# Cappucciyes/ViT-With-OpenCL

Measured on AMD Instinct MI355X. Metric: images/sec ViT-B/16 224x224 bs512, higher is better.
Workload: dtype f32

## Files before the change

### include/kernelHandler.h

```cpp
#ifndef VIT_HIP_KERNELHANDLER_H
#define VIT_HIP_KERNELHANDLER_H

#include <stddef.h>
#include <stdio.h>
#include <stdlib.h>

#ifdef __cplusplus
extern "C" {
#endif

typedef void *vh_stream_t;
typedef void *vh_event_t;

#define VH_CHECK(err)                                                          \
    do {                                                                       \
        int vh_check_err_ = (err);                                             \
        if (vh_check_err_ != 0) {                                              \
            printf("[%s:%d] HIP error %d: %s\n", __FILE__, __LINE__,           \
                   vh_check_err_, vh_last_error());                            \
            exit(EXIT_FAILURE);                                                \
        }                                                                      \
    } while (0)

int vh_device_count(void);
// ... 89 lines not shown
int vh_launch_attention_planes_f16(vh_stream_t s, const void *qkv_planes_f16, void *output, int output_planes,
                                   int n_images, int tokens, int embed_dim, int num_heads);
int vh_launch_attention_planes_f16_hd80(vh_stream_t s, const void *qkv_planes_f16, float *output, int n_images,
                                        int tokens, int embed_dim, int num_heads);
int vh_launch_attention_planes_f16_hd80_operand(vh_stream_t s, const void *qkv_planes_f16, void *output, void *out_scales,
                                                int output_kind, int n_images, int tokens, int embed_dim, int num_heads);
int vh_launch_attention_long(vh_stream_t s, const void *qkv_planes, int parts, float *output, int n_images, int tokens,
                             int embed_dim, int num_heads);
int vh_launch_linear_p3(vh_stream_t s, void *output, int output_planes, const void *weight_planes,
                        const void *input_planes, const float *bias, int rowA, int colA, int colB,
                        int doGelu, const float *residual);
int vh_launch_linear_p3_cols(vh_stream_t s, void *output, int output_planes, const void *weight_planes, int w_features,
                             const void *input_planes, const float *bias, int rowA, int colA, int colB);
int vh_launch_attention_planes_cls(vh_stream_t s, const void *qkv_planes, const void *q_cls_planes, void *out_cls_planes,
                                   int n_images, int tokens, int embed_dim, int num_heads);

int vh_launch_split2h_planes(vh_stream_t s, const float *weight, void *planes, int rows, int cols, float scale);
int vh_launch_linear_h2(vh_stream_t s, float *output, const void *weight_planes, float weight_scale,
                        const float *input, const float *bias, int rowA, int colA, int colB,
                        int doGelu, const float *residual);
int vh_launch_attention_h2(vh_stream_t s, const float *qkv, float *output, int n_images, int tokens,
                           int embed_dim, int num_heads);

int vh_launch_attention(vh_stream_t s, const float *qkv, float *output, int n_images,
                        int tokens, int embed_dim, int num_heads);
enum { VH_ATTN_NATIVE = 0, VH_ATTN_FP16 = 1, VH_ATTN_FP16X2 = 2, VH_ATTN_SPLIT3 = 3 };
enum { VH_ATTN_AUTO = 0, VH_ATTN_STREAMING = 1 };
int vh_launch_attention_rows(vh_stream_t s, const float *qkv, void *output, int out_kind, int arith, int kernel, int n_images,
                             int tokens, int embed_dim, int num_heads);

// ... 168 lines not shown
```

### vit-with-opencl_amd/csrc/ViT_hip.c

```c
#include "ViT_opencl.h"
#include "kernel_limits.h"
#include "vit_ingest.h"
#include "vit_multi.h"
#include "vit_pipeline.h"
#include "vit_plan.h"
#include "vit_planes_file.h"
#include "vit_requests.h"

#include <math.h>
#include <stdint.h>
#include <stdio.h>
#include <stdlib.h>
#include <string.h>
#include <time.h>

#define TRY(expr)                 \
    do {                          \
        int try_rc_ = (expr);     \
        if (try_rc_ != 0) {       \
            rc = try_rc_;         \
            goto fail;            \
        }                         \
    } while (0)

// ... 558 lines not shown
    return rc;
}

static int layer_f32_planes_attention(vit_hip_ctx *ctx, vh_stream_t s, int n, int l, int timed)
{
    int rc = 0;
    const vit_config *c = &ctx->cfg;
    const int E = c->embed_dim, T = ctx->plan.tokens, rows = n * T, fold = ctx->plan.ln_fold;
    float **lw = layer_tensors(ctx, l);
    const struct operand *op = ctx->op + 4 * l;
    const int planes_attn = ctx->plan.qkv_form == VH_QKV_PLANES3;
    OP_T(timed, VIT_OP_QKV, fold ? vh_launch_linear_p3_norm(s, ctx->qkv, planes_attn, op[0].w, ctx->y, ctx->stats, op[0].colsum, op[0].bias_folded, c->eps, rows, E, 3 * E, 0)
                                 : vh_launch_linear_p3(s, ctx->qkv, planes_attn, op[0].w, ctx->y, lw[3], rows, E, 3 * E, 0, NULL));
    if (timed)
        TRY(attention_tap(ctx, s, n, l));
    OP_T(timed, VIT_OP_ATTENTION, ctx->plan.attn_form == ATTN_HD64 ? vh_launch_attention_planes(s, ctx->qkv, ctx->attn, n, T, E, c->num_heads)
                                  : (rc = ctx->plan.attn_form == ATTN_LONG ? vh_launch_attention_long(s, ctx->qkv, 3, ctx->hid, n, T, E, c->num_heads)
                                                                      : attention_rows(ctx, s, ctx->hid, VH_ATTN_SPLIT3, n)) != 0 ? rc
                                  : vh_launch_split3_rows(s, ctx->hid, ctx->attn, rows, E));
    return 0;
fail:
    return rc;
}

static int layer_f32_planes_tail(vit_hip_ctx *ctx, vh_stream_t s, int n, int l, int timed)
{
    int rc = 0;
    const vit_config *c = &ctx->cfg;
    const int E = c->embed_dim, F = c->mlp_hidden, rows = n * ctx->plan.tokens, fold = ctx->plan.ln_fold, last = l == c->depth - 1;
    float **lw = layer_tensors(ctx, l);
    const struct operand *op = ctx->op + 4 * l;
// ... 44 lines not shown
    if (!fold)
        OP(VIT_OP_LAYER_NORM, vh_launch_layer_norm_p3(s, ctx->x, lw[0], lw[1], ctx->y, rows, E, E, c->eps));
    if (last && cls_only) {
        size_t off[3], q_off;
        plan_cls_only_scratch(c, n, off);
        plan_cls_query_scratch(c, n, &q_off);
        char *scratch = (char *)ctx->qkv;
        float *x_cls = (float *)scratch;
        char *attn_cls = scratch + off[0], *y_cls = scratch + off[1], *hid_cls = scratch + off[2], *q_cls = scratch + q_off;
        const int cls_query = ctx->plan.cls_query && !attention_tap_reads(ctx, l);
        if (cls_query) {
            char *kv = scratch + (size_t)rows * E * 6;
            OP(VIT_OP_QKV, (rc = vh_launch_linear_p3_cols(s, kv, 1, (const char *)op[0].w + (size_t)E * 64, 3 * E, ctx->y, lw[3] + E, rows, E, 2 * E)) != 0 ? rc :
                           (rc = vh_launch_gather_rows(s, ctx->y, y_cls, 3 * (E / 32), rows, n, 64, T)) != 0 ? rc :
                           vh_launch_linear_p3_cols(s, q_cls, 1, op[0].w, 3 * E, y_cls, lw[3], n, E, E));
            OP(VIT_OP_ATTENTION, vh_launch_attention_planes_cls(s, ctx->qkv, q_cls, attn_cls, n, T, E, c->num_heads));
        } else {
            TRY(layer_f32_planes_attention(ctx, s, n, l, 1));
        }
        OP(VIT_OP_OUT_PROJ_CLS, (rc = cls_query ? 0 : vh_launch_gather_rows(s, ctx->attn, attn_cls, 3 * (E / 32), rows, n, 64, T)) != 0 ? rc :
                                (rc = vh_launch_gather_rows(s, ctx->x, x_cls, 1, rows, n, 4 * E, T)) != 0 ? rc :
                                vh_launch_linear_p3(s, x_cls, 0, op[1].w, attn_cls, lw[5], n, E, E, 0, x_cls));
        OP(VIT_OP_LAYER_NORM, vh_launch_layer_norm_p3(s, x_cls, lw[6], lw[7], y_cls, n, E, E, c->eps));
        OP(VIT_OP_FC1_CLS, vh_launch_linear_p3(s, hid_cls, 1, op[2].w, y_cls, lw[9], n, E, F, 1, NULL));
        OP(VIT_OP_FC2_CLS, vh_launch_linear_p3(s, x_cls, 0, op[3].w, hid_cls, lw[11], n, F, E, 0, x_cls));
        *cls_rows = cls_query ? 2 : 1;
        return 0;
    }
    TRY(layer_f32_planes_attention(ctx, s, n, l, 1));
    return layer_f32_planes_tail(ctx, s, n, l, 1);
fail:
// ... 771 lines not shown
```

### vit-with-opencl_amd/csrc/attention_p3.hip

```cpp
#include "kernelHandler.h"
#include "kernel_limits.h"
#include "vit_kernels.h"
#include "fp32_split.h"
#include "gemm_common.h"

namespace {

constexpr int HD = 64;
constexpr int MAX_LDS = KL_LDS_BYTES;
constexpr int MAX_ROWS = KL_ATTN_HD64_MAX_TOKENS;
static_assert(2 * 2 * 3 * MAX_ROWS * 64 <= MAX_LDS && MAX_ROWS % 16 == 0 && MAX_ROWS <= 32 * 7, "the rows of launch_k and launch_t");

typedef const __attribute__((address_space(1))) void *gptr_t;
typedef __attribute__((address_space(3))) void *lptr_t;
typedef short s16x4 __attribute__((ext_vector_type(4)));

template <int NKT, int NPL, int OUTK, bool CLSQ = false>
__global__ __launch_bounds__(64 * NKT) void attention_p3_kernel(const char *__restrict__ qkv3, char *__restrict__ out3,
                                                               unsigned char *__restrict__ aux,
                                                               int T, int E, int H, int n_items, int RB)
{
    static_assert((NPL == 3 && OUTK == 3) || (NPL == 1 && (OUTK == 4 || OUTK == 0 || OUTK == 8)), "parts / output kind");
    static_assert(!CLSQ || OUTK == 3, "the class-query variant runs on the exact planes");
    unsigned char *const out_scales = aux;
    typedef typename PartT<NPL>::type part_t;
    constexpr int NT = NPL == 3 ? 6 : 1;
    extern __shared__ __attribute__((aligned(16))) char smem[];
    const int slot = 2 * NPL * RB * 64;
    char *Kb = smem, *Vb = smem + slot;

    const int tid = threadIdx.x, lane = tid & 63;
    const int wave = __builtin_amdgcn_readfirstlane(tid >> 6);
    const int lr = lane & 31, lh = lane >> 5;
    const int E32 = E >> 5, rb16 = RB >> 4, pieces = 2 * NPL * rb16;
    const size_t prow = (size_t)(n_items / H) * T;
// ... 99 lines not shown
                        __builtin_amdgcn_sched_group_barrier(0x008, 2, 0);
                    }
                    __builtin_amdgcn_sched_barrier(0);
                }
            }
        }

        __syncthreads();
        if (next < n_items) {
            dma(next, 1, Kb);
            if (computes)
                load_q(next);
        }

        if (computes) {
#pragma unroll
            for (int r = 0; r < 16; ++r) {
                const int key = 32 * (NKT - 1) + (r & 3) + 8 * (r >> 2) + 4 * lh;
                s[NKT - 1][r] = key < T ? s[NKT - 1][r] : -INFINITY;
            }
            float mx = -INFINITY;
#pragma unroll
            for (int j = 0; j < NKT; ++j)
#pragma unroll
                for (int r = 0; r < 16; ++r)
                    mx = fmaxf(mx, s[j][r]);
            mx = fmaxf(mx, __shfl_xor(mx, 32));
            const float c1 = 1.44269504088896340736f / sqrtf((float)HD);
            const float c2 = -mx * c1;
            float sum = 0.0f;
#pragma unroll
            for (int j = 0; j < NKT; ++j)
#pragma unroll
                for (int r = 0; r < 16; ++r) {
                    const float e = __builtin_amdgcn_exp2f(__builtin_fmaf(s[j][r], c1, c2));
                    s[j][r] = e;
                    sum += e;
                }
            sum += __shfl_xor(sum, 32);
            const float inv_sum = 1.0f / sum;
#pragma unroll
            for (int j = 0; j < NKT; ++j)
#pragma unroll
                for (int r = 0; r < 16; ++r)
                    s[j][r] = s[j][r] * inv_sum;

            f32x16 o[2];
#pragma unroll
            for (int r = 0; r < 16; ++r) {
                o[0][r] = 0.0f;
                o[1][r] = 0.0f;
            }
            part_t vq[2][NPL], pp[NPL];
            auto read_v = [&](part_t (&v3)[NPL], int f) {
                const int j = f >> 2, t = (f >> 1) & 1, dt = f & 1;
                const int r0 = (j == NKT - 1) ? min(32 * j + 16 * t, RB - 16) : 32 * j + 16 * t;
#pragma unroll
                for (int o3 = 0; o3 < NPL; ++o3) {
                    const int pl = (NPL - o3) % NPL;
                    const char *vp = Vb + (dt * NPL + pl) * RB * 64 + r0 * 64 + vofs;
                    const s16x4 lo = __builtin_amdgcn_ds_read_tr16_b64_v4i16((__attribute__((address_space(3))) s16x4 *)(vp));
                    const s16x4 hi = __builtin_amdgcn_ds_read_tr16_b64_v4i16((__attribute__((address_space(3))) s16x4 *)(vp + 8 * 64));
                    typedef short s16x8 __attribute__((ext_vector_type(8)));
                    v3[pl] = __builtin_bit_cast(part_t, s16x8{lo[0], lo[1], lo[2], lo[3], hi[0], hi[1], hi[2], hi[3]});
                }
            };
            read_v(vq[0], 0);
#pragma unroll
            for (int f = 0; f < 4 * NKT; ++f) {
                const int j = f >> 2, t = (f >> 1) & 1, dt = f & 1;
                if (f + 1 < 4 * NKT)
                    read_v(vq[(f + 1) & 1], f + 1);
                if (dt == 0)
                    split_parts(f32x4{s[j][8 * t], s[j][8 * t + 1], s[j][8 * t + 2], s[j][8 * t + 3]},
                                f32x4{s[j][8 * t + 4], s[j][8 * t + 5], s[j][8 * t + 6], s[j][8 * t + 7]}, pp);
                if (!(j == NKT - 1 && 32 * j + 16 * t >= T)) {
#pragma unroll
                    for (int tt = 0; tt < NT; ++tt)
                        o[dt] = mfma_part(vq[f & 1][term_w<NPL>(tt)], pp[term_a<NPL>(tt)], o[dt]);
                }
            }

            if (CLSQ ? lr == 0 : q < T) {
                typedef unsigned u32x2 __attribute__((ext_vector_type(2)));
                typedef unsigned u32x4 __attribute__((ext_vector_type(4)));
                constexpr int OPL = OUTK == 3 ? 3 : 1;
#pragma unroll
                for (int dt = 0; dt < 2; ++dt) {
                    if (OUTK == 0) {
                        float *row = reinterpret_cast<float *>(out3) + ((size_t)b * T + q) * E + h * HD + 32 * dt + 4 * lh;
// ... 46 lines not shown
                    for (int pl = 0; pl < OPL; ++pl)
#pragma unroll
                        for (int g = 0; g < 4; g += 2) {
                            const auto r0 = __builtin_amdgcn_permlane32_swap(pg[g][pl][0], pg[g + 1][pl][0], false, false);
                            const auto r1 = __builtin_amdgcn_permlane32_swap(pg[g][pl][1], pg[g + 1][pl][1], false, false);
                            *reinterpret_cast<u32x4 *>(d3 + (size_t)pl * orows * 64 + 16 * g) = u32x4{r0[0], r1[0], r0[1], r1[1]};
                        }
                }
            }
        }

        __syncthreads();
    }
}

template <int NKT, int NPL, int OUTK, bool CLSQ>
int launch_k(hipStream_t st, const char *qkv3, char *out3, unsigned char *aux, int n_images, int T, int E, int H)
{
    const int RB = (T + 15) / 16 * 16;
    const size_t lds = (size_t)2 * 2 * NPL * RB * 64;
    VH_SET_LDS_ONCE((attention_p3_kernel<NKT, NPL, OUTK, CLSQ>), MAX_LDS);
    const int num_cus = vh_device_cus(vh_current_device());
    const int n_items = n_images * H;
    const int grid = n_items < num_cus ? n_items : num_cus;
    hipLaunchKernelGGL((attention_p3_kernel<NKT, NPL, OUTK, CLSQ>), dim3(grid), dim3(64 * NKT), lds, st, qkv3, out3, aux, T, E, H, n_items, RB);
    VH_LAUNCH_CHECK("attention_p3_kernel");
    return 0;
}


template <int NPL, int OUTK, bool CLSQ = false>
int launch_t(hipStream_t st, const char *in, char *out, unsigned char *out_scales, int n_images, int tokens, int embed_dim, int num_heads)
{
    switch ((tokens + 31) / 32) {
    case 1: return launch_k<1, NPL, OUTK, CLSQ>(st, in, out, out_scales, n_images, tokens, embed_dim, num_heads);
    case 2: return launch_k<2, NPL, OUTK, CLSQ>(st, in, out, out_scales, n_images, tokens, embed_dim, num_heads);
    case 3: return launch_k<3, NPL, OUTK, CLSQ>(st, in, out, out_scales, n_images, tokens, embed_dim, num_heads);
    case 4: return launch_k<4, NPL, OUTK, CLSQ>(st, in, out, out_scales, n_images, tokens, embed_dim, num_heads);
    case 5: return launch_k<5, NPL, OUTK, CLSQ>(st, in, out, out_scales, n_images, tokens, embed_dim, num_heads);
    case 6: return launch_k<6, NPL, OUTK, CLSQ>(st, in, out, out_scales, n_images, tokens, embed_dim, num_heads);
    default: return launch_k<7, NPL, OUTK, CLSQ>(st, in, out, out_scales, n_images, tokens, embed_dim, num_heads);
    }
}

int check_args(const char *who, const void *in, const void *out, int n_images, int tokens, int embed_dim, int num_heads)
{
    if (!in || !out)
        return vh_fail(1, "%s: null pointer argument", who);
    if (n_images <= 0 || tokens <= 0 || num_heads <= 0 || embed_dim != num_heads * HD || tokens > MAX_ROWS)
        return vh_fail(1, "%s: needs head_dim 64 and 1 <= tokens <= %d (n=%d tokens=%d embed=%d heads=%d)", who,
                       MAX_ROWS, n_images, tokens, embed_dim, num_heads);
    if ((((uintptr_t)in | (uintptr_t)out) & 15) != 0)
        return vh_fail(1, "%s: pointers must be 16-byte aligned", who);
    return 0;
}

// ... 7 lines not shown
    return launch_t<3, 3>((hipStream_t)s, static_cast<const char *>(qkv_planes), static_cast<char *>(out_planes), nullptr,
                          n_images, tokens, embed_dim, num_heads);
}

extern "C" int vh_launch_attention_planes_cls(vh_stream_t s, const void *qkv_planes, const void *q_cls_planes, void *out_cls_planes,
                                              int n_images, int tokens, int embed_dim, int num_heads)
{
    if (int rc = check_args("vh_launch_attention_planes_cls", qkv_planes, out_cls_planes, n_images, tokens, embed_dim, num_heads))
        return rc;
    if (!q_cls_planes || ((uintptr_t)q_cls_planes & 15) != 0)
        return vh_fail(1, "vh_launch_attention_planes_cls: q_cls_planes must be a 16-byte aligned pointer");
    return launch_t<3, 3, true>((hipStream_t)s, static_cast<const char *>(qkv_planes), static_cast<char *>(out_cls_planes),
                                static_cast<unsigned char *>(const_cast<void *>(q_cls_planes)), n_images, tokens, embed_dim, num_heads);
}

extern "C" int vh_launch_attention_planes_f16(vh_stream_t s, const void *qkv_planes_f16, void *output, int output_planes,
                                              int n_images, int tokens, int embed_dim, int num_heads)
{
    if (int rc = check_args("vh_launch_attention_planes_f16", qkv_planes_f16, output, n_images, tokens, embed_dim, num_heads))
        return rc;
    const char *in = static_cast<const char *>(qkv_planes_f16);
    char *out = static_cast<char *>(output);
    return output_planes ? launch_t<1, 4>((hipStream_t)s, in, out, nullptr, n_images, tokens, embed_dim, num_heads)
                         : launch_t<1, 0>((hipStream_t)s, in, out, nullptr, n_images, tokens, embed_dim, num_heads);
}

extern "C" int vh_launch_attention_planes_f16_mx(vh_stream_t s, const void *qkv_planes_f16, void *out_values, void *out_scales,
                                                 int n_images, int tokens, int embed_dim, int num_heads)
{
    if (int rc = check_args("vh_launch_attention_planes_f16_mx", qkv_planes_f16, out_values, n_images, tokens, embed_dim, num_heads))
// ... 7 lines not shown
```

### vit-with-opencl_amd/csrc/kernel_limits.h

```cpp
#ifndef VIT_KERNEL_LIMITS_H
#define VIT_KERNEL_LIMITS_H

#include "kernelHandler.h"

#include <stddef.h>

#ifdef __cplusplus
#define KL_FN static constexpr
#else
#define KL_FN static inline
#endif

enum { KL_LDS_BYTES = 160 * 1024 };

enum {
    KL_ATTN_HD64_MAX_TOKENS = 208,
    KL_ATTN_HD80_MAX_TOKENS = 272,
    KL_ATTN_STREAMING_MAX_TOKENS = 512
};
KL_FN int kl_attn_long_head_dim_ok(int head_dim) { return head_dim == 64 || head_dim == 80; }

enum { KL_LN_PLANES_ROWS = 16, KL_LN_PLANES_MAX_EMBED = 2048 };
KL_FN int kl_layer_norm_planes_max_embed(int parts)
{
    if (parts != 1 && parts != 3)
        return 0;
    const int by_lds = KL_LDS_BYTES / (parts * KL_LN_PLANES_ROWS * 64) * 32;
    return by_lds < KL_LN_PLANES_MAX_EMBED ? by_lds : KL_LN_PLANES_MAX_EMBED;
}

enum { KL_FOLD_GROUP = 128, KL_FOLD_MAX_GROUPS = 16 };

enum {
// ... 89 lines not shown
```

### vit-with-opencl_amd/csrc/vit_plan.c

```c
#include "vit_plan.h"
#include "vit_ingest.h"
#include "kernel_limits.h"

#include <stdio.h>
#include <stdlib.h>
#include <string.h>

void plan_env_parse(struct plan_env *env, const char *const v[PLAN_ENV_COUNT])
{
    const char *const p = v[PLAN_ENV_PRECISION], *const fold = v[PLAN_ENV_LN_FOLD], *const attn = v[PLAN_ENV_ATTN];
    env->precision = (p && p[0] == 'b') ? VIT_PRECISION_BF16_GEMM
                   : (p && strncmp(p, "fp16x2", 6) == 0) ? VIT_PRECISION_F32_FP16X2
                   : (p && strncmp(p, "fp8", 3) == 0) ? VIT_PRECISION_FP8_GEMM : VIT_PRECISION_F32;
    env->p3_off = v[PLAN_ENV_P3] && v[PLAN_ENV_P3][0] == '0';
    env->fp32_native = v[PLAN_ENV_GEMM_FP32] && v[PLAN_ENV_GEMM_FP32][0] == 'n';
    env->ln_fold = (fold && fold[0] == '0') ? 0 : (fold && fold[0] == '1') ? 1 : -1;
    env->last_layer_cls = v[PLAN_ENV_LAST_LAYER] && strcmp(v[PLAN_ENV_LAST_LAYER], "cls") == 0;
    env->last_layer_full = v[PLAN_ENV_LAST_LAYER] && strcmp(v[PLAN_ENV_LAST_LAYER], "full") == 0;
    env->last_layer_all_queries = v[PLAN_ENV_LAST_LAYER] && strcmp(v[PLAN_ENV_LAST_LAYER], "all_queries") == 0;
    env->attn_long = attn && strcmp(attn, "long") == 0;
    env->attn_tiled = attn && attn[0] == 't';
}

void plan_env_read(struct plan_env *env)
{
    const char *const values[PLAN_ENV_COUNT] = {getenv("VIT_HIP_PRECISION"), getenv("VIT_HIP_P3"), getenv("VIT_HIP_GEMM_FP32"),
                                                getenv("VIT_HIP_LN_FOLD"), getenv("VIT_HIP_LAST_LAYER"), getenv("VIT_HIP_ATTN")};
    plan_env_parse(env, values);
}

static size_t max_of(size_t a, size_t b) { return a > b ? a : b; }

size_t plan_cls_only_scratch(const vit_config *cfg, int n, size_t off[3])
{
    const size_t rows = (size_t)n, E = (size_t)cfg->embed_dim, F = (size_t)cfg->mlp_hidden;
    size_t o[3];
    o[0] = align_up(rows * E * 4, 256);
    o[1] = o[0] + align_up(rows * E * 6, 256);
    o[2] = o[1] + align_up(rows * E * 6, 256);
    if (off)
        memcpy(off, o, sizeof o);
    return o[2] + rows * F * 6;
}
// ... 158 lines not shown
    plan->qkv_form = plan->attn_form == ATTN_STREAMING ? VH_QKV_ROWS_F32 : reduced ? VH_QKV_PLANES_F16 : VH_QKV_PLANES3;
    plan->weight_planes = weight_planes;
    plan->operand_bytes = precision == VIT_PRECISION_BF16_GEMM ? 2 : precision == VIT_PRECISION_FP8_GEMM ? 1
                        : precision == VIT_PRECISION_F32_FP16X2 ? 4 : weight_planes ? 6 : 0;
    plan->operand_scales = precision == VIT_PRECISION_FP8_GEMM;
    plan->conv_parts = reduced ? 1 : weight_planes ? 3 : 0;
    plan->planes_patch_embed = plan->ln_fold || use_p3 || reduced;
    plan->act_bytes = use_p3 ? 6 : (int)sizeof(float);
    plan_layout(plan, cfg, NULL, NULL, NULL, plan->slab_bytes);
    plan_arena(plan, cfg, max_batch);
    plan->cls_only_ok = use_p3 && !ln_fold && T >= 4 && plan_cls_only_scratch(cfg, max_batch, NULL) <= plan->qkv_bytes;
    plan->last_layer_lazy = plan->cls_only_ok && !env->last_layer_full;
    plan->cls_query = plan->last_layer_lazy && !env->last_layer_all_queries && plan->attn_form == ATTN_HD64 &&
                      plan->qkv_form == VH_QKV_PLANES3 &&
                      22 * (size_t)E + 6 * (size_t)F + 5 * 256 <= (size_t)T * (size_t)E * 6;
    return 0;
}
```

### vit-with-opencl_amd/csrc/vit_plan.h

```cpp
#ifndef VIT_PLAN_H
#define VIT_PLAN_H

#include "ViT_opencl.h"

#include <stddef.h>

struct operand
{
    void *w;
    void *scales;
    float pair_scale;
    float *colsum, *bias_folded;
};

enum { SLAB_F32, SLAB_OPERAND, SLAB_CONV, SLAB_FOLD, N_SLABS };

enum { ATTN_STREAMING, ATTN_HD64, ATTN_HD80, ATTN_LONG };

enum { MAX_DEPTH = 256, MAX_TENSORS = 4 + 12 * MAX_DEPTH + 4 };

static inline int plan_operand_tensor(int m)
{
    static const int big[4] = {2, 4, 8, 10};
    return 4 + 12 * (m / 4) + big[m % 4];
}

struct plan_env
{
    int precision;
    int p3_off;
    int fp32_native;
    int ln_fold;
    int last_layer_cls;
    int last_layer_full;
    int last_layer_all_queries;
    int attn_long;
    int attn_tiled;
};
enum { PLAN_ENV_PRECISION, PLAN_ENV_P3, PLAN_ENV_GEMM_FP32, PLAN_ENV_LN_FOLD, PLAN_ENV_LAST_LAYER, PLAN_ENV_ATTN, PLAN_ENV_COUNT };
void plan_env_parse(struct plan_env *env, const char *const values[PLAN_ENV_COUNT]);
void plan_env_read(struct plan_env *env);

struct vit_plan
{
    int precision;
    int ln_fold;
    int use_p3;
    int cls_only_last;
    int attn_form;
    int fp32_native;
    int attn_rows_streaming;
    int tokens;
    int qkv_form;
    int weight_planes;
    int operand_bytes;
    int operand_scales;
    int conv_parts;
    int planes_patch_embed;
    int act_bytes;
    int cls_only_ok;
    int last_layer_lazy;
    int cls_query;
    size_t slab_bytes[N_SLABS];
    size_t x_bytes, y_bytes, attn_bytes, qkv_bytes, ws_bytes, stats_bytes;
    size_t crop_off;
    size_t e_scales_off, hid_scales_off;
};

int plan_make(struct vit_plan *plan, const vit_config *cfg, int n_tensors, int max_batch, int precision, int ln_fold,
              const struct plan_env *env);

void plan_layout(const struct vit_plan *plan, const vit_config *cfg, void *const slabs[N_SLABS], float **w, struct operand *op,
                 size_t bytes[N_SLABS]);

size_t plan_cls_only_scratch(const vit_config *cfg, int n, size_t off[3]);
size_t plan_cls_query_scratch(const vit_config *cfg, int n, size_t *q_off);

// ... 2 lines not shown
```

### vit-with-opencl_amd/host/abi.py

```python
from __future__ import annotations

import ctypes as C

P = C.POINTER
i, u, l, sz, ull, f, d = C.c_int, C.c_uint, C.c_long, C.c_size_t, C.c_ulonglong, C.c_float, C.c_double
p, s = C.c_void_p, C.c_char_p
voidp = p
f32p = fp = P(f)
pp, fpp, ip, lp, dp, szp, u8p = P(p), P(fp), P(i), P(l), P(d), P(sz), P(C.c_ubyte)

STRUCTS = {}
ENUMS = []


def mirrors(ctype: str):
    def register(cls):
        STRUCTS[ctype] = cls
        return cls
    return register


def enum(prefix: str, mapping: dict, names: dict | None = None) -> dict:
    ENUMS.append((prefix, mapping, names))
    return mapping


FP32_MATH = enum("VH_FP32_", {"split3": 0, "native": 1})
ATTN_ARITH = enum("VH_ATTN_", {"native": 0, "fp16": 1, "fp16x2": 2, "split3": 3})
ATTN_KERNEL = enum("VH_ATTN_", {"auto": 0, "streaming": 1})
QKV_FORMS = enum("VH_QKV_", {"rows_f32": 0, "planes3": 1, "planes_f16": 2})
TOPK_SCORES = enum("VIT_TOPK_", {"probs": 0, "logits": 1})
GALLERY_DTYPES = enum("VH_GALLERY_", {"f32": 0, "bf16": 1})
GALLERY_MAX_SPLITS, GALLERY_ROW_TILE = 1024, 128
enum("VH_GALLERY_", {"max_splits": GALLERY_MAX_SPLITS, "row_tile": GALLERY_ROW_TILE})
DENSE_MAX_LABELS, DENSE_MAX_GRID, DENSE_TOKEN_TILE = 256, 64, 128
enum("VH_DENSE_", {"max_labels": DENSE_MAX_LABELS, "max_grid": DENSE_MAX_GRID, "token_tile": DENSE_TOKEN_TILE})
STITCH_BLOCK, STITCH_MAX_SIDE = 16, 16384
enum("VH_STITCH_", {"block": STITCH_BLOCK, "max_side": STITCH_MAX_SIDE})
POS_MODES = enum("VH_POS_", {"bicubic": 0, "bilinear": 1})
enum("VIT_POS_", POS_MODES)

PRECISIONS = enum("VIT_PRECISION_", {"f32": 0, "bf16": 1, "fp8": 2, "f32_fp16x2": 3},
                  names={"bf16": "VIT_PRECISION_BF16_GEMM", "fp8": "VIT_PRECISION_FP8_GEMM"})
PIXEL_LAYOUTS = enum("VIT_PIXELS_", {"hwc": 0, "chw": 1})
# ... 197 lines not shown
        _fn("vh_launch_merge_rows", p, p, p, i, i, i),
        _fn("vh_layer_norm_planes_max_embed", i),
        _fn("vh_launch_layer_norm_planes", p, p, p, p, p, i, i, i, l, d),
        _fn("vh_launch_attention_planes_bf16", p, p, p, i, i, i, i),
        _fn("vh_launch_linear_planes", p, p, i, p, p, i, p, i, i, i, i, p),
        _fn("vh_launch_layer_norm_p3", p, p, p, p, p, i, i, l, d),
        _fn("vh_launch_attention_p3", p, p, p, i, i, i, i),
        _fn("vh_launch_attention_planes", p, p, p, i, i, i, i),
        _fn("vh_launch_attention_planes_f16", p, p, p, i, i, i, i, i),
        _fn("vh_launch_attention_planes_f16_hd80", p, p, p, i, i, i, i),
        _fn("vh_launch_attention_planes_f16_hd80_operand", p, p, p, p, i, i, i, i, i),
        _fn("vh_launch_attention_long", p, p, i, p, i, i, i, i),
        _fn("vh_launch_linear_p3", p, p, i, p, p, p, i, i, i, i, p),
        _fn("vh_launch_linear_p3_cols", p, p, i, p, i, p, p, i, i, i),
        _fn("vh_launch_attention_planes_cls", p, p, p, p, i, i, i, i),
        _fn("vh_launch_split2h_planes", p, p, p, i, i, f),
        _fn("vh_launch_linear_h2", p, p, p, f, p, p, i, i, i, i, p),
        _fn("vh_launch_attention_h2", p, p, p, i, i, i, i),
        _fn("vh_launch_attention", p, p, p, i, i, i, i),
        _fn("vh_launch_attention_rows", p, p, p, i, i, i, i, i, i, i),
        _fn("vh_launch_gather_rows", p, p, p, i, i, i, i, i),
        _fn("vh_launch_softmax", p, p, p, i, i),
        _fn("vh_launch_topk", p, p, i, i, i, i, p, p),
        _fn("vh_cls_attention_head_dim_ok", i),
        _fn("vh_launch_cls_attention", p, p, i, i, i, i, i, i, i, p, p),
        _fn("vh_rollout_workspace", i, i, ret=sz),
        _fn("vh_rollout_max_tokens", i),
        _fn("vh_launch_rollout_step", p, p, i, i, i, i, i, p, p, p),
        _fn("vh_launch_rollout_read", p, p, i, i, p),
        _fn("vh_launch_attention_f16", p, p, p, i, i, i, i),
# ... 149 lines not shown
```

Before: 6529.

## Skip masked key groups in attention softmax and add one-wave CLS attention kernel

Attention softmax now checks the count of live keys in the last 32-key tile and skips max, exp, scale and split work for groups that are fully past the token count. This is the default path unless VIT_HIP_ATTN_MASKED=all is set. A new single-wave persistent kernel handles the last layer's class-token query. It stages V through LDS with transposed reads and prefetches the next head, and it becomes the default unless VIT_HIP_CLS_ATTN=workgroup is set. The change cuts wasted ALU work on padded keys and over-provisioned workgroups for the CLS-only layer, at the cost of more code paths and branches.

```diff
diff --git a/include/kernelHandler.h b/include/kernelHandler.h
--- a/include/kernelHandler.h
+++ b/include/kernelHandler.h
@@ -127,6 +127,12 @@
                              const void *input_planes, const float *bias, int rowA, int colA, int colB);
 int vh_launch_attention_planes_cls(vh_stream_t s, const void *qkv_planes, const void *q_cls_planes, void *out_cls_planes,
                                    int n_images, int tokens, int embed_dim, int num_heads);
+enum {
+    VH_ATTN_CLS_WORKGROUP = 1,
+    VH_ATTN_EVERY_GROUP = 2
+};
+int vh_launch_attention_planes_forms(vh_stream_t s, const void *qkv_planes, const void *q_cls_planes, void *out_planes,
+                                     int n_images, int tokens, int embed_dim, int num_heads, unsigned forms);
 
 int vh_launch_split2h_planes(vh_stream_t s, const float *weight, void *planes, int rows, int cols, float scale);
 int vh_launch_linear_h2(vh_stream_t s, float *output, const void *weight_planes, float weight_scale,
diff --git a/vit-with-opencl_amd/csrc/ViT_hip.c b/vit-with-opencl_amd/csrc/ViT_hip.c
--- a/vit-with-opencl_amd/csrc/ViT_hip.c
+++ b/vit-with-opencl_amd/csrc/ViT_hip.c
@@ -596,7 +596,7 @@
                                  : vh_launch_linear_p3(s, ctx->qkv, planes_attn, op[0].w, ctx->y, lw[3], rows, E, 3 * E, 0, NULL));
     if (timed)
         TRY(attention_tap(ctx, s, n, l));
-    OP_T(timed, VIT_OP_ATTENTION, ctx->plan.attn_form == ATTN_HD64 ? vh_launch_attention_planes(s, ctx->qkv, ctx->attn, n, T, E, c->num_heads)
+    OP_T(timed, VIT_OP_ATTENTION, ctx->plan.attn_form == ATTN_HD64 ? vh_launch_attention_planes_forms(s, ctx->qkv, NULL, ctx->attn, n, T, E, c->num_heads, ctx->plan.attn_forms)
                                   : (rc = ctx->plan.attn_form == ATTN_LONG ? vh_launch_attention_long(s, ctx->qkv, 3, ctx->hid, n, T, E, c->num_heads)
                                                                       : attention_rows(ctx, s, ctx->hid, VH_ATTN_SPLIT3, n)) != 0 ? rc
                                   : vh_launch_split3_rows(s, ctx->hid, ctx->attn, rows, E));
@@ -671,7 +671,7 @@
             OP(VIT_OP_QKV, (rc = vh_launch_linear_p3_cols(s, kv, 1, (const char *)op[0].w + (size_t)E * 64, 3 * E, ctx->y, lw[3] + E, rows, E, 2 * E)) != 0 ? rc :
                            (rc = vh_launch_gather_rows(s, ctx->y, y_cls, 3 * (E / 32), rows, n, 64, T)) != 0 ? rc :
                            vh_launch_linear_p3_cols(s, q_cls, 1, op[0].w, 3 * E, y_cls, lw[3], n, E, E));
-            OP(VIT_OP_ATTENTION, vh_launch_attention_planes_cls(s, ctx->qkv, q_cls, attn_cls, n, T, E, c->num_heads));
+            OP(VIT_OP_ATTENTION, vh_launch_attention_planes_forms(s, ctx->qkv, q_cls, attn_cls, n, T, E, c->num_heads, ctx->plan.attn_forms));
         } else {
             TRY(layer_f32_planes_attention(ctx, s, n, l, 1));
         }
diff --git a/vit-with-opencl_amd/csrc/attention_p3.hip b/vit-with-opencl_amd/csrc/attention_p3.hip
--- a/vit-with-opencl_amd/csrc/attention_p3.hip
+++ b/vit-with-opencl_amd/csrc/attention_p3.hip
@@ -4,6 +4,8 @@
 #include "fp32_split.h"
 #include "gemm_common.h"
 
+#include <utility>
+
 namespace {
 
 constexpr int HD = 64;
@@ -15,10 +17,96 @@
 typedef __attribute__((address_space(3))) void *lptr_t;
 typedef short s16x4 __attribute__((ext_vector_type(4)));
 
+template <int NKT>
+__device__ __forceinline__ void softmax_columns(f32x16 (&s)[NKT], int T, int lh, int live)
+{
+    constexpr int L = NKT - 1;
+    const float c1 = 1.44269504088896340736f / sqrtf((float)HD);
+    float mx = -INFINITY;
+    auto mask_max = [&](int g) {
+#pragma unroll
+        for (int r = 4 * g; r < 4 * g + 4; ++r) {
+            const int key = 32 * L + (r & 3) + 8 * (r >> 2) + 4 * lh;
+            s[L][r] = key < T ? s[L][r] : -INFINITY;
+            mx = fmaxf(mx, s[L][r]);
+        }
+    };
+#pragma unroll
+    for (int j = 0; j < L; ++j)
+#pragma unroll
+        for (int r = 0; r < 16; ++r)
+            mx = fmaxf(mx, s[j][r]);
+    mask_max(0);
+    if (8 < live) {
+        mask_max(1);
+        if (16 < live) {
+            mask_max(2);
+            if (24 < live)
+                mask_max(3);
+        }
+    }
+    mx = fmaxf(mx, __shfl_xor(mx, 32));
+    const float c2 = -mx * c1;
+    float sum = 0.0f;
+    auto exp_sum = [&](int j, int g) {
+#pragma unroll
+        for (int r = 4 * g; r < 4 * g + 4; ++r) {
+            const float e = __builtin_amdgcn_exp2f(__builtin_fmaf(s[j][r], c1, c2));
+            s[j][r] = e;
+            sum += e;
+        }
+    };
+#pragma unroll
+    for (int j = 0; j < L; ++j)
+#pragma unroll
+        for (int g = 0; g < 4; ++g)
+            exp_sum(j, g);
+    exp_sum(L, 0);
+    if (8 < live) {
+        exp_sum(L, 1);
+        if (16 < live) {
+            exp_sum(L, 2);
+            if (24 < live)
+                exp_sum(L, 3);
+        }
+    }
+    sum += __shfl_xor(sum, 32);
+    const float inv_sum = 1.0f / sum;
+    auto scale = [&](int j, int g) {
+#pragma unroll
+        for (int r = 4 * g; r < 4 * g + 4; ++r)
+            s[j][r] = s[j][r] * inv_sum;
+    };
+#pragma unroll
+    for (int j = 0; j < L; ++j)
+#pragma unroll
+        for (int g = 0; g < 4; ++g)
+            scale(j, g);
+    scale(L, 0);
+    if (8 < live) {
+        scale(L, 1);
+        if (16 < live) {
+            scale(L, 2);
+            if (24 < live)
+                scale(L, 3);
+        }
+    }
+}
+
+template <int NKT, int NPL>
+__device__ __forceinline__ void split_p(const f32x16 (&s)[NKT], int j, int t, int live, typename PartT<NPL>::type (&pp)[NPL])
+{
+    const f32x4 lo = f32x4{s[j][8 * t], s[j][8 * t + 1], s[j][8 * t + 2], s[j][8 * t + 3]};
+    if (j == NKT - 1 && 8 * (2 * t + 1) >= live)
+        split_parts(lo, f32x4{0.0f, 0.0f, 0.0f, 0.0f}, pp);
+    else
+        split_parts(lo, f32x4{s[j][8 * t + 4], s[j][8 * t + 5], s[j][8 * t + 6], s[j][8 * t + 7]}, pp);
+}
+
 template <int NKT, int NPL, int OUTK, bool CLSQ = false>
 __global__ __launch_bounds__(64 * NKT) void attention_p3_kernel(const char *__restrict__ qkv3, char *__restrict__ out3,
                                                                unsigned char *__restrict__ aux,
-                                                               int T, int E, int H, int n_items, int RB)
+                                                               int T, int E, int H, int n_items, int RB, int live)
 {
     static_assert((NPL == 3 && OUTK == 3) || (NPL == 1 && (OUTK == 4 || OUTK == 0 || OUTK == 8)), "parts / output kind");
     static_assert(!CLSQ || OUTK == 3, "the class-query variant runs on the exact planes");
@@ -148,36 +236,7 @@
         }
 
         if (computes) {
-#pragma unroll
-            for (int r = 0; r < 16; ++r) {
-                const int key = 32 * (NKT - 1) + (r & 3) + 8 * (r >> 2) + 4 * lh;
-                s[NKT - 1][r] = key < T ? s[NKT - 1][r] : -INFINITY;
-            }
-            float mx = -INFINITY;
-#pragma unroll
-            for (int j = 0; j < NKT; ++j)
-#pragma unroll
-                for (int r = 0; r < 16; ++r)
-                    mx = fmaxf(mx, s[j][r]);
-            mx = fmaxf(mx, __shfl_xor(mx, 32));
-            const float c1 = 1.44269504088896340736f / sqrtf((float)HD);
-            const float c2 = -mx * c1;
-            float sum = 0.0f;
-#pragma unroll
-            for (int j = 0; j < NKT; ++j)
-#pragma unroll
-                for (int r = 0; r < 16; ++r) {
-                    const float e = __builtin_amdgcn_exp2f(__builtin_fmaf(s[j][r], c1, c2));
-                    s[j][r] = e;
-                    sum += e;
-                }
-            sum += __shfl_xor(sum, 32);
-            const float inv_sum = 1.0f / sum;
-#pragma unroll
-            for (int j = 0; j < NKT; ++j)
-#pragma unroll
-                for (int r = 0; r < 16; ++r)
-                    s[j][r] = s[j][r] * inv_sum;
+            softmax_columns<NKT>(s, T, lh, live);
 
             f32x16 o[2];
 #pragma unroll
@@ -205,9 +264,8 @@
                 const int j = f >> 2, t = (f >> 1) & 1, dt = f & 1;
                 if (f + 1 < 4 * NKT)
                     read_v(vq[(f + 1) & 1], f + 1);
-                if (dt == 0)
-                    split_parts(f32x4{s[j][8 * t], s[j][8 * t + 1], s[j][8 * t + 2], s[j][8 * t + 3]},
-                                f32x4{s[j][8 * t + 4], s[j][8 * t + 5], s[j][8 * t + 6], s[j][8 * t + 7]}, pp);
+                if (dt == 0 && !(j == NKT - 1 && 16 * t >= live))
+                    split_p<NKT, NPL>(s, j, t, live, pp);
                 if (!(j == NKT - 1 && 32 * j + 16 * t >= T)) {
 #pragma unroll
                     for (int tt = 0; tt < NT; ++tt)
@@ -284,32 +342,232 @@
     }
 }
 
+template <class F, int... I>
+__device__ __forceinline__ void static_for_each(F &&f, std::integer_sequence<int, I...>)
+{
+    (f(std::integral_constant<int, I>{}), ...);
+}
+template <int N, class F>
+__device__ __forceinline__ void static_for(F &&f)
+{
+    static_for_each(f, std::make_integer_sequence<int, N>{});
+}
+
+constexpr int CW_LDS = KL_ATTN_CLS_WAVE_LDS_BYTES;
+static_assert(CW_LDS == 2 * 3 * 32 * 64, "one 32-key tile of V: [d tile][part][32 rows][64 B]");
+
+template <int NKT>
+__global__ __launch_bounds__(64) void attention_p3_cls_wave_kernel(const char *__restrict__ qkv3, char *__restrict__ out3,
+                                                                   const char *__restrict__ qcls, int T, int E, int H,
+                                                                   int n_items, int live)
+{
+    constexpr int NPL = 3, NT = 6, NF = NKT * (HD / 16);
+    constexpr int KR = NF < 7 ? NF + 1 : 7;
+    constexpr int VR = NKT < 2 ? NKT : 2;
+    typedef bf16x8 part_t;
+    __shared__ __attribute__((aligned(16))) char vtile[CW_LDS];
+
+    const int lane = threadIdx.x, lr = lane & 31, lh = lane >> 5;
+    const int E32 = E >> 5;
+    const size_t orows = (size_t)(n_items / H), prow = orows * T;
+    const int vofs = (4 * lh + ((lane & 15) >> 2)) * 64 + ((lane & 16) + 4 * (lane & 3)) * 2;
+
+    f32x4 qraw[HD / 16][NPL];
+    auto load_q = [&](int it) {
+        const int b = it / H, h = it - b * H;
+#pragma unroll
+        for (int g = 0; g < HD / 16; ++g)
+#pragma unroll
+            for (int pl = 0; pl < NPL; ++pl)
+                qraw[g][pl] = *reinterpret_cast<const f32x4 *>(
+                    qcls + ((size_t)((2 * h + (g >> 1)) * NPL + pl) * orows + b) * 64 + 16 * (2 * (g & 1) + lh));
+    };
+    part_t kp[KR][NPL];
+    auto load_k = [&](part_t (&k3)[NPL], int it, int f) {
+        const int b = it / H, h = it - b * H;
+        const int j = f / (HD / 16), g = f % (HD / 16);
+        const size_t row = (size_t)b * T + min(32 * j + lr, T - 1);
+#pragma unroll
+        for (int o = 0; o < NPL; ++o) {
+            const int pl = (NPL - o) % NPL;
+            k3[pl] = __builtin_bit_cast(part_t, *reinterpret_cast<const f32x4 *>(
+                         qkv3 + ((size_t)((E32 + 2 * h + (g >> 1)) * NPL + pl) * prow + row) * 64 + 16 * (2 * (g & 1) + lh)));
+        }
+    };
+    auto load_head = [&](int it) {
+        load_q(it);
+#pragma unroll
+        for (int f = 0; f < KR - 1; ++f)
+            load_k(kp[f], it, f);
+    };
+
+    int item = blockIdx.x;
+    load_head(item);
+    for (;;) {
+        const int b = item / H, h = item - b * H;
+        const int next = item + (int)gridDim.x;
+
+        part_t qp[HD / 16][NPL];
+#pragma unroll
+        for (int g = 0; g < HD / 16; ++g)
+#pragma unroll
+            for (int pl = 0; pl < NPL; ++pl)
+                qp[g][pl] = __builtin_bit_cast(part_t, lr == 0 ? qraw[g][pl] : f32x4{0.0f, 0.0f, 0.0f, 0.0f});
+
+        f32x16 s[NKT];
+#pragma unroll
+        for (int f = 0; f < NF; ++f) {
+            const int j = f / (HD / 16), g = f % (HD / 16);
+            if (g == 0) {
+#pragma unroll
+                for (int r = 0; r < 16; ++r)
+                    s[j][r] = 0.0f;
+            }
+            if (f + KR - 1 < NF)
+                load_k(kp[(f + KR - 1) % KR], item, f + KR - 1);
+            __builtin_amdgcn_sched_barrier(0);
+#pragma unroll
+            for (int t = 0; t < NT; ++t)
+                s[j] = mfma_part(kp[f % KR][term_w<NPL>(t)], qp[g][term_a<NPL>(t)], s[j]);
+            __builtin_amdgcn_sched_barrier(0);
+        }
+
+        f32x4 vst[VR][12];
+        auto load_v = [&](int j) {
+#pragma unroll
+            for (int p = 0; p < 12; ++p) {
+                const int r = 32 * j + 16 * (p & 1) + (lane >> 2);
+                vst[j % VR][p] = *reinterpret_cast<const f32x4 *>(
+                    qkv3 + ((size_t)((2 * E32 + 2 * h) * NPL + (p >> 1)) * prow + (size_t)b * T + min(r, T - 1)) * 64 + 16 * (lane & 3));
+            }
+        };
+        auto store_v = [&](int j) {
+#pragma unroll
+            for (int p = 0; p < 12; ++p)
+                *reinterpret_cast<f32x4 *>(vtile + p * 1024 + lane * 16) = vst[j % VR][p];
+        };
+#pragma unroll
+        for (int j = 0; j < VR; ++j)
+            load_v(j);
+        load_head(next < n_items ? next : item);
+        __builtin_amdgcn_sched_barrier(0);
+
+        softmax_columns<NKT>(s, T, lh, live);
+
+        f32x16 o[2];
+#pragma unroll
+        for (int r = 0; r < 16; ++r) {
+            o[0][r] = 0.0f;
+            o[1][r] = 0.0f;
+        }
+        part_t vq[2][NPL], pp[NPL];
+        auto read_v = [&](part_t (&v3)[NPL], int f) {
+            const int t = (f >> 1) & 1, dt = f & 1;
+#pragma unroll
+            for (int o3 = 0; o3 < NPL; ++o3) {
+                const int pl = (NPL - o3) % NPL;
+                const char *vp = vtile + (dt * NPL + pl) * 2048 + 16 * t * 64 + vofs;
+                const s16x4 lo = __builtin_amdgcn_ds_read_tr16_b64_v4i16((__attribute__((address_space(3))) s16x4 *)(vp));
+                const s16x4 hi = __builtin_amdgcn_ds_read_tr16_b64_v4i16((__attribute__((address_space(3))) s16x4 *)(vp + 8 * 64));
+                typedef short s16x8 __attribute__((ext_vector_type(8)));
+                v3[pl] = __builtin_bit_cast(part_t, s16x8{lo[0], lo[1], lo[2], lo[3], hi[0], hi[1], hi[2], hi[3]});
+            }
+        };
+        store_v(0);
+        if (VR < NKT)
+            load_v(VR);
+        read_v(vq[0], 0);
+        static_for<4 * NKT>([&](auto step) __attribute__((always_inline)) {
+            constexpr int f = decltype(step)::value, j = f >> 2, t = (f >> 1) & 1, dt = f & 1;
+            if (f + 1 < 4 * NKT) {
+                if ((f & 3) == 3) {
+                    store_v(j + 1);
+                    if (j + 1 + VR < NKT)
+                        load_v(j + 1 + VR);
+                }
+                read_v(vq[(f + 1) & 1], f + 1);
+            }
+            if (dt == 0 && !(j == NKT - 1 && 16 * t >= live))
+                split_p<NKT, NPL>(s, j, t, live, pp);
+            if (!(j == NKT - 1 && 32 * j + 16 * t >= T)) {
+#pragma unroll
+                for (int tt = 0; tt < NT; ++tt)
+                    o[dt] = mfma_part(vq[f & 1][term_w<NPL>(tt)], pp[term_a<NPL>(tt)], o[dt]);
+            }
+        });
+
+        if (lr == 0) {
+            typedef unsigned u32x2 __attribute__((ext_vector_type(2)));
+            typedef unsigned u32x4 __attribute__((ext_vector_type(4)));
+#pragma unroll
+            for (int dt = 0; dt < 2; ++dt) {
+                u32x2 pg[4][NPL];
+#pragma unroll
+                for (int g = 0; g < 4; ++g) {
+                    bf16x4 part[3];
+                    split4(f32x4{o[dt][4 * g], o[dt][4 * g + 1], o[dt][4 * g + 2], o[dt][4 * g + 3]}, part[0], part[1], part[2]);
+#pragma unroll
+                    for (int pl = 0; pl < NPL; ++pl)
+                        pg[g][pl] = __builtin_bit_cast(u32x2, part[pl]);
+                }
+                char *d3 = out3 + ((size_t)(2 * h + dt) * NPL * orows + (size_t)b) * 64 + 16 * lh;
+#pragma unroll
+                for (int pl = 0; pl < NPL; ++pl)
+#pragma unroll
+                    for (int g = 0; g < 4; g += 2) {
+                        const auto r0 = __builtin_amdgcn_permlane32_swap(pg[g][pl][0], pg[g + 1][pl][0], false, false);
+                        const auto r1 = __builtin_amdgcn_permlane32_swap(pg[g][pl][1], pg[g + 1][pl][1], false, false);
+                        *reinterpret_cast<u32x4 *>(d3 + (size_t)pl * orows * 64 + 16 * g) = u32x4{r0[0], r1[0], r0[1], r1[1]};
+                    }
+            }
+        }
+        if (next >= n_items)
+            break;
+        item = next;
+    }
+}
+
+template <int NKT>
+int launch_cls_wave(hipStream_t st, const char *qkv3, char *out3, const char *qcls, int n_images, int T, int E, int H, int live)
+{
+    const int n_items = n_images * H, waves = vh_device_cus(vh_current_device()) * KL_ATTN_CLS_WAVES_PER_CU;
+    hipLaunchKernelGGL((attention_p3_cls_wave_kernel<NKT>), dim3(n_items < waves ? n_items : waves), dim3(64), 0, st, qkv3, out3, qcls,
+                       T, E, H, n_items, live);
+    VH_LAUNCH_CHECK("attention_p3_cls_wave_kernel");
+    return 0;
+}
+
 template <int NKT, int NPL, int OUTK, bool CLSQ>
-int launch_k(hipStream_t st, const char *qkv3, char *out3, unsigned char *aux, int n_images, int T, int E, int H)
-{
+int launch_k(hipStream_t st, const char *qkv3, char *out3, unsigned char *aux, int n_images, int T, int E, int H, unsigned forms)
+{
+    const int live = (forms & VH_ATTN_EVERY_GROUP) ? 32 : T - 32 * (NKT - 1);
+    if constexpr (CLSQ)
+        if (!(forms & VH_ATTN_CLS_WORKGROUP))
+            return launch_cls_wave<NKT>(st, qkv3, out3, reinterpret_cast<const char *>(aux), n_images, T, E, H, live);
     const int RB = (T + 15) / 16 * 16;
     const size_t lds = (size_t)2 * 2 * NPL * RB * 64;
     VH_SET_LDS_ONCE((attention_p3_kernel<NKT, NPL, OUTK, CLSQ>), MAX_LDS);
     const int num_cus = vh_device_cus(vh_current_device());
     const int n_items = n_images * H;
     const int grid = n_items < num_cus ? n_items : num_cus;
-    hipLaunchKernelGGL((attention_p3_kernel<NKT, NPL, OUTK, CLSQ>), dim3(grid), dim3(64 * NKT), lds, st, qkv3, out3, aux, T, E, H, n_items, RB);
+    hipLaunchKernelGGL((attention_p3_kernel<NKT, NPL, OUTK, CLSQ>), dim3(grid), dim3(64 * NKT), lds, st, qkv3, out3, aux, T, E, H, n_items, RB, live);
     VH_LAUNCH_CHECK("attention_p3_kernel");
     return 0;
 }
 
 
 template <int NPL, int OUTK, bool CLSQ = false>
-int launch_t(hipStream_t st, const char *in, char *out, unsigned char *out_scales, int n_images, int tokens, int embed_dim, int num_heads)
+int launch_t(hipStream_t st, const char *in, char *out, unsigned char *out_scales, int n_images, int tokens, int embed_dim, int num_heads,
+             unsigned forms = 0)
 {
     switch ((tokens + 31) / 32) {
-    case 1: return launch_k<1, NPL, OUTK, CLSQ>(st, in, out, out_scales, n_images, tokens, embed_dim, num_heads);
-    case 2: return launch_k<2, NPL, OUTK, CLSQ>(st, in, out, out_scales, n_images, tokens, embed_dim, num_heads);
-    case 3: return launch_k<3, NPL, OUTK, CLSQ>(st, in, out, out_scales, n_images, tokens, embed_dim, num_heads);
-    case 4: return launch_k<4, NPL, OUTK, CLSQ>(st, in, out, out_scales, n_images, tokens, embed_dim, num_heads);
-    case 5: return launch_k<5, NPL, OUTK, CLSQ>(st, in, out, out_scales, n_images, tokens, embed_dim, num_heads);
-    case 6: return launch_k<6, NPL, OUTK, CLSQ>(st, in, out, out_scales, n_images, tokens, embed_dim, num_heads);
-    default: return launch_k<7, NPL, OUTK, CLSQ>(st, in, out, out_scales, n_images, tokens, embed_dim, num_heads);
+    case 1: return launch_k<1, NPL, OUTK, CLSQ>(st, in, out, out_scales, n_images, tokens, embed_dim, num_heads, forms);
+    case 2: return launch_k<2, NPL, OUTK, CLSQ>(st, in, out, out_scales, n_images, tokens, embed_dim, num_heads, forms);
+    case 3: return launch_k<3, NPL, OUTK, CLSQ>(st, in, out, out_scales, n_images, tokens, embed_dim, num_heads, forms);
+    case 4: return launch_k<4, NPL, OUTK, CLSQ>(st, in, out, out_scales, n_images, tokens, embed_dim, num_heads, forms);
+    case 5: return launch_k<5, NPL, OUTK, CLSQ>(st, in, out, out_scales, n_images, tokens, embed_dim, num_heads, forms);
+    case 6: return launch_k<6, NPL, OUTK, CLSQ>(st, in, out, out_scales, n_images, tokens, embed_dim, num_heads, forms);
+    default: return launch_k<7, NPL, OUTK, CLSQ>(st, in, out, out_scales, n_images, tokens, embed_dim, num_heads, forms);
     }
 }
 
@@ -347,6 +605,21 @@
                                 static_cast<unsigned char *>(const_cast<void *>(q_cls_planes)), n_images, tokens, embed_dim, num_heads);
 }
 
+extern "C" int vh_launch_attention_planes_forms(vh_stream_t s, const void *qkv_planes, const void *q_cls_planes, void *out_planes,
+                                                int n_images, int tokens, int embed_dim, int num_heads, unsigned forms)
+{
+    if (int rc = check_args("vh_launch_attention_planes_forms", qkv_planes, out_planes, n_images, tokens, embed_dim, num_heads))
+        return rc;
+    if (((uintptr_t)q_cls_planes & 15) != 0 || (forms & ~(unsigned)(VH_ATTN_CLS_WORKGROUP | VH_ATTN_EVERY_GROUP)) != 0)
+        return vh_fail(1, "vh_launch_attention_planes_forms: q_cls_planes must be 16-byte aligned and forms a set of VH_ATTN_* (%u)", forms);
+    const char *in = static_cast<const char *>(qkv_planes);
+    char *out = static_cast<char *>(out_planes);
+    if (!q_cls_planes)
+        return launch_t<3, 3>((hipStream_t)s, in, out, nullptr, n_images, tokens, embed_dim, num_heads, forms);
+    return launch_t<3, 3, true>((hipStream_t)s, in, out, static_cast<unsigned char *>(const_cast<void *>(q_cls_planes)), n_images, tokens,
+                                embed_dim, num_heads, forms);
+}
+
 extern "C" int vh_launch_attention_planes_f16(vh_stream_t s, const void *qkv_planes_f16, void *output, int output_planes,
                                               int n_images, int tokens, int embed_dim, int num_heads)
 {
diff --git a/vit-with-opencl_amd/csrc/kernel_limits.h b/vit-with-opencl_amd/csrc/kernel_limits.h
--- a/vit-with-opencl_amd/csrc/kernel_limits.h
+++ b/vit-with-opencl_amd/csrc/kernel_limits.h
@@ -17,6 +17,12 @@
     KL_ATTN_HD64_MAX_TOKENS = 208,
     KL_ATTN_HD80_MAX_TOKENS = 272,
     KL_ATTN_STREAMING_MAX_TOKENS = 512
+};
+enum {
+    KL_ATTN_CLS_WAVE_LDS_BYTES = 2 * 3 * 32 * 64,
+    KL_SIMDS_PER_CU = 4,
+    KL_ATTN_CLS_WAVES_PER_CU = KL_LDS_BYTES / KL_ATTN_CLS_WAVE_LDS_BYTES < KL_SIMDS_PER_CU ? KL_LDS_BYTES / KL_ATTN_CLS_WAVE_LDS_BYTES
+                                                                                           : KL_SIMDS_PER_CU
 };
 KL_FN int kl_attn_long_head_dim_ok(int head_dim) { return head_dim == 64 || head_dim == 80; }
 
diff --git a/vit-with-opencl_amd/csrc/vit_plan.c b/vit-with-opencl_amd/csrc/vit_plan.c
--- a/vit-with-opencl_amd/csrc/vit_plan.c
+++ b/vit-with-opencl_amd/csrc/vit_plan.c
@@ -20,13 +20,22 @@
     env->last_layer_all_queries = v[PLAN_ENV_LAST_LAYER] && strcmp(v[PLAN_ENV_LAST_LAYER], "all_queries") == 0;
     env->attn_long = attn && strcmp(attn, "long") == 0;
     env->attn_tiled = attn && attn[0] == 't';
+    env->cls_attn_workgroup = env->attn_masked_all = 0;
+}
+
+void plan_env_parse_forms(struct plan_env *env, const char *const v[PLAN_FORM_COUNT])
+{
+    env->cls_attn_workgroup = v[PLAN_FORM_CLS_ATTN] && strcmp(v[PLAN_FORM_CLS_ATTN], "workgroup") == 0;
+    env->attn_masked_all = v[PLAN_FORM_ATTN_MASKED] && strcmp(v[PLAN_FORM_ATTN_MASKED], "all") == 0;
 }
 
 void plan_env_read(struct plan_env *env)
 {
     const char *const values[PLAN_ENV_COUNT] = {getenv("VIT_HIP_PRECISION"), getenv("VIT_HIP_P3"), getenv("VIT_HIP_GEMM_FP32"),
                                                 getenv("VIT_HIP_LN_FOLD"), getenv("VIT_HIP_LAST_LAYER"), getenv("VIT_HIP_ATTN")};
+    const char *const forms[PLAN_FORM_COUNT] = {getenv("VIT_HIP_CLS_ATTN"), getenv("VIT_HIP_ATTN_MASKED")};
     plan_env_parse(env, values);
+    plan_env_parse_forms(env, forms);
 }
 
 static size_t max_of(size_t a, size_t b) { return a > b ? a : b; }
@@ -215,5 +224,8 @@
     plan->cls_query = plan->last_layer_lazy && !env->last_layer_all_queries && plan->attn_form == ATTN_HD64 &&
                       plan->qkv_form == VH_QKV_PLANES3 &&
                       22 * (size_t)E + 6 * (size_t)F + 5 * 256 <= (size_t)T * (size_t)E * 6;
+    if (plan->attn_form == ATTN_HD64 && plan->qkv_form == VH_QKV_PLANES3)
+        plan->attn_forms = (plan->cls_query && env->cls_attn_workgroup ? VH_ATTN_CLS_WORKGROUP : 0u) |
+                           (env->attn_masked_all ? VH_ATTN_EVERY_GROUP : 0u);
     return 0;
 }
diff --git a/vit-with-opencl_amd/csrc/vit_plan.h b/vit-with-opencl_amd/csrc/vit_plan.h
--- a/vit-with-opencl_amd/csrc/vit_plan.h
+++ b/vit-with-opencl_amd/csrc/vit_plan.h
@@ -36,9 +36,13 @@
     int last_layer_all_queries;
     int attn_long;
     int attn_tiled;
+    int cls_attn_workgroup;
+    int attn_masked_all;
 };
 enum { PLAN_ENV_PRECISION, PLAN_ENV_P3, PLAN_ENV_GEMM_FP32, PLAN_ENV_LN_FOLD, PLAN_ENV_LAST_LAYER, PLAN_ENV_ATTN, PLAN_ENV_COUNT };
 void plan_env_parse(struct plan_env *env, const char *const values[PLAN_ENV_COUNT]);
+enum { PLAN_FORM_CLS_ATTN, PLAN_FORM_ATTN_MASKED, PLAN_FORM_COUNT };
+void plan_env_parse_forms(struct plan_env *env, const char *const values[PLAN_FORM_COUNT]);
 void plan_env_read(struct plan_env *env);
 
 struct vit_plan
@@ -61,6 +65,7 @@
     int cls_only_ok;
     int last_layer_lazy;
     int cls_query;
+    unsigned attn_forms;
     size_t slab_bytes[N_SLABS];
     size_t x_bytes, y_bytes, attn_bytes, qkv_bytes, ws_bytes, stats_bytes;
     size_t crop_off;
diff --git a/vit-with-opencl_amd/host/abi.py b/vit-with-opencl_amd/host/abi.py
--- a/vit-with-opencl_amd/host/abi.py
+++ b/vit-with-opencl_amd/host/abi.py
@@ -28,6 +28,7 @@
 FP32_MATH = enum("VH_FP32_", {"split3": 0, "native": 1})
 ATTN_ARITH = enum("VH_ATTN_", {"native": 0, "fp16": 1, "fp16x2": 2, "split3": 3})
 ATTN_KERNEL = enum("VH_ATTN_", {"auto": 0, "streaming": 1})
+ATTN_FORMS = enum("VH_ATTN_", {"cls_workgroup": 1, "every_group": 2})
 QKV_FORMS = enum("VH_QKV_", {"rows_f32": 0, "planes3": 1, "planes_f16": 2})
 TOPK_SCORES = enum("VIT_TOPK_", {"probs": 0, "logits": 1})
 GALLERY_DTYPES = enum("VH_GALLERY_", {"f32": 0, "bf16": 1})
@@ -255,6 +256,7 @@
         _fn("vh_launch_linear_p3", p, p, i, p, p, p, i, i, i, i, p),
         _fn("vh_launch_linear_p3_cols", p, p, i, p, i, p, p, i, i, i),
         _fn("vh_launch_attention_planes_cls", p, p, p, p, i, i, i, i),
+        _fn("vh_launch_attention_planes_forms", p, p, p, p, i, i, i, i, u),
         _fn("vh_launch_split2h_planes", p, p, p, i, i, f),
         _fn("vh_launch_linear_h2", p, p, p, f, p, p, i, i, i, i, p),
         _fn("vh_launch_attention_h2", p, p, p, i, i, i, i),
```

New measurement: 6544 (median of 6 runs). Within noise of the previous version (+0.2%).
